# fernandezdaniel/MOBOCMF

Measured on AMD Instinct MI355X. Metric: ELBO steps/sec (MFDGP d=8 M=512 N=8192 S=8), higher is better.
Workload: dtype f64

## Files before the change

### mobocmf_amd/csrc/gram.hip

```cpp
#include "common.h"

#define GT 128
#define GM 32


typedef double v2f64_t __attribute__((ext_vector_type(2)));

template <int KIND, int DB, int XD>
__global__ __launch_bounds__(GT) void gram_fwd_kernel(GramArgs g) {
    __shared__ __attribute__((aligned(16))) double stg[XD ? (GT / 64) * 64 * (XD + 2) : 1];
    __shared__ double zs[GM][DB];
    __shared__ double zfs[GM];
    __shared__ double il1[DB], il2[DB];
    const int d = g.d;
    const int tid = threadIdx.x;
    const int gm = g.gm;
    const int m0 = blockIdx.y * gm;
    const double* hyp = g.hyp;
    double a1, af = 0, nu = 0, a2 = 0, ilf = 0;
    if (KIND == 0) {
        a1 = hyp[0];
        if (tid < DB) il1[tid] = tid < d ? 1.0 / hyp[1 + tid] : 0.0;
    } else {
        a1 = hyp[0]; af = hyp[1]; nu = hyp[2]; a2 = hyp[3]; ilf = 1.0 / hyp[4];
        if (tid < DB) { il1[tid] = tid < d ? 1.0 / hyp[5 + tid] : 0.0; il2[tid] = tid < d ? 1.0 / hyp[5 + d + tid] : 0.0; }
    }
    for (int e = tid; e < gm * DB; e += GT) {
        int mm = e / DB, k = e % DB;
        int m = m0 + mm;
        zs[mm][k] = (m < g.M && k < d) ? g.Zx[(int64_t)(m / g.zdiv) * d + k] : 0.0;
    }
    if (KIND == 1 && tid < gm) zfs[tid] = (m0 + tid < g.M) ? g.zf[m0 + tid] : 0.0;
    __syncthreads();

    const int64_t n0 = (int64_t)blockIdx.x * GT + tid;
    const int xdiv = XD ? XD : g.xdiv;
    const int64_t c0 = n0 * xdiv;
    if (c0 >= g.Np) return;
    const bool real = n0 < g.nbase;
    double xr[DB];
#pragma unroll
    for (int k = 0; k < DB; ++k) xr[k] = (real && k < d) ? g.x[n0 * d + k] : 0.0;
    double fr[XD ? XD : 1];
    if (XD && KIND == 1) {
#pragma unroll
        for (int s = 0; s < XD; s += 2) {
            v2f64_t v = real ? *(const v2f64_t*)(g.f + c0 + s) : (v2f64_t){0.0, 0.0};
            fr[s] = v[0];
            fr[s + 1] = v[1];
        }
    }

    const bool full_wave = XD && __ballot(real) == ~0ull;
    (void)full_wave;
    if (g.knn && blockIdx.y == 0) {
        for (int s = 0; s < xdiv; ++s) {
            int64_t n = c0 + s;
            if (n >= g.Np) break;
            double v = 0.0;
            if (real) {
                if (KIND == 0) v = a1;
                else { double fn = g.f[n]; v = a1 * (nu * fn * fn + af) + a2; }
            }
            g.knn[n] = v;
        }
    }
    for (int mm = 0; mm < gm; ++mm) {
        const int m = m0 + mm;
        double* krow = g.K + (int64_t)m * g.ldk;
        if (!real || m >= g.M) {
            for (int s = 0; s < xdiv; ++s) {
                int64_t n = c0 + s;
                if (n >= g.Np) break;
                krow[n] = (g.is_kmm && n == m) ? 1.0 : 0.0;
            }
            continue;
        }
        double d1 = 0.0, d2 = 0.0;
#pragma unroll
        for (int k = 0; k < DB; ++k) {
            double df = xr[k] - zs[mm][k];
            double t1 = df * il1[k];
            d1 += t1 * t1;
            if (KIND == 1) { double t2 = df * il2[k]; d2 += t2 * t2; }
        }
        const double E1 = exp(-0.5 * d1);
        if (KIND == 0) {
            double v = a1 * E1;
            if (g.is_kmm && c0 == m) v += g.jitter;
            krow[c0] = v;
            for (int s = 1; s < xdiv; ++s) krow[c0 + s] = a1 * E1;
        } else if (XD) {
            const double E2 = exp(-0.5 * d2);
            const double zfm = zfs[mm];
            const double c1 = a1 * E1, c2 = a2 * E2;
            const double cp = c1 * nu * zfm, cq = c1 * af;
            const int lane = tid & 63;
            double* my = stg + (tid >> 6) * 64 * (XD + 2);
#pragma unroll
            for (int s = 0; s < XD; s += 2) {
                v2f64_t v;
#pragma unroll
                for (int e = 0; e < 2; ++e) {
                    const double fn = fr[s + e];
                    const double fd = (fn - zfm) * ilf;
                    v[e] = cq * exp(-0.5 * fd * fd) + (cp * fn + c2);
                }
                if (full_wave) *(v2f64_t*)(my + lane * (XD + 2) + s) = v;
                else *(v2f64_t*)(krow + c0 + s) = v;
            }
            if (full_wave) {
                double* wrow = krow + (c0 - (int64_t)lane * XD);
#pragma unroll
                for (int i = 0; i < XD / 2; ++i) {
                    const int e = (i * 64 + lane) * 2;
                    *(v2f64_t*)(wrow + e) = *(const v2f64_t*)(my + (e / XD) * (XD + 2) + e % XD);
                }
            }
        } else {
            const double E2 = exp(-0.5 * d2);
            const double zfm = zfs[mm];
            const double c1 = a1 * E1, c2 = a2 * E2;
            for (int s = 0; s < xdiv; ++s) {
                const int64_t n = c0 + s;
                const double fn = g.f[n];
                const double fd = (fn - zfm) * ilf;
                const double Ef = exp(-0.5 * fd * fd);
                double v = c1 * (nu * fn * zfm + af * Ef) + c2;
                if (g.is_kmm && n == m) v += g.jitter;
                krow[n] = v;
            }
        }
    }
}

__device__ __forceinline__ double wave_sum(double v) {
    v += __shfl_xor(v, 1);
    v += __shfl_xor(v, 2);
    v += __shfl_xor(v, 4);
    v += __shfl_xor(v, 8);
    v += __shfl_xor(v, 16);
    v += __shfl_xor(v, 32);
    return v;
}

template <int KIND, int DB, bool WANT_DX, int XD>
__global__ __launch_bounds__(GT) void gram_bwd_kernel(GramArgs g) {
    __shared__ double zs[GM][DB];
    __shared__ double zfs[GM];
    __shared__ double il1[DB], il2[DB];
    __shared__ double dzf_s[GM];
    __shared__ double red[2][8 + 2 * DB];
    extern __shared__ double dfs[];
    const int d = g.d;
    const int tid = threadIdx.x, lane = tid & 63, wave = tid >> 6;
    const int gm = g.gm;
    const int m0 = blockIdx.y * gm;
    const double* hyp = g.hyp;
    double a1, af = 0, nu = 0, a2 = 0, ilf = 0;
    if (KIND == 0) {
        a1 = hyp[0];
        if (tid < DB) il1[tid] = tid < d ? 1.0 / hyp[1 + tid] : 0.0;
    } else {
        a1 = hyp[0]; af = hyp[1]; nu = hyp[2]; a2 = hyp[3]; ilf = 1.0 / hyp[4];
        if (tid < DB) { il1[tid] = tid < d ? 1.0 / hyp[5 + tid] : 0.0; il2[tid] = tid < d ? 1.0 / hyp[5 + d + tid] : 0.0; }
    }
    for (int e = tid; e < gm * DB; e += GT) {
        int mm = e / DB, k = e % DB;
        int m = m0 + mm;
        zs[mm][k] = (m < g.M && k < d) ? g.Zx[(int64_t)(m / g.zdiv) * d + k] : 0.0;
    }
    if (tid < gm) {
        dzf_s[tid] = 0.0;
        if (KIND == 1) zfs[tid] = (m0 + tid < g.M) ? g.zf[m0 + tid] : 0.0;
    }
    __syncthreads();

    const int64_t n0 = (int64_t)blockIdx.x * GT + tid;
    const int xdiv = XD ? XD : g.xdiv;
    const int64_t c0 = n0 * xdiv;
    const bool real = n0 < g.nbase;
    static_assert(XD == 0 || 128 % XD == 0, "replica runs must not straddle a column block");
    unsigned long long amask = ~0ull;
    if (g.colact && real) {
        if (XD) amask = g.colact[c0 >> 7] != 0 ? ~0ull : 0ull;
        else {
            amask = 0ull;
            for (int s = 0; s < xdiv; ++s) amask |= (unsigned long long)(g.colact[(c0 + s) >> 7] != 0 ? 1 : 0) << s;
        }
    }
    const bool live = real && amask != 0ull;
    double fr[XD ? XD : 1], dfa[XD ? XD : 1];
    if (XD) {
#pragma unroll
        for (int s = 0; s < XD; s += 2) {
            v2f64_t v = real ? *(const v2f64_t*)(g.f + c0 + s) : (v2f64_t){0.0, 0.0};
            fr[s] = v[0];
            fr[s + 1] = v[1];
            dfa[s] = dfa[s + 1] = 0.0;
        }
    }
    double xr[DB], aL1[DB], aL2[KIND == 1 ? DB : 1], aX[WANT_DX ? DB : 1];
#pragma unroll
    for (int k = 0; k < DB; ++k) {
        xr[k] = (real && k < d) ? g.x[n0 * d + k] : 0.0;
        aL1[k] = 0.0;
        if (KIND == 1) aL2[k] = 0.0;
        if (WANT_DX) aX[k] = 0.0;
    }
    double s_a1 = 0, s_af = 0, s_nu = 0, s_a2 = 0, s_lsf = 0;
    if (KIND == 1 && !XD)
        for (int s = 0; s < xdiv; ++s) dfs[s * GT + tid] = 0.0;

    if (g.gknn && blockIdx.y == 0 && real) {
        for (int s = 0; s < xdiv; ++s) {
            const int64_t n = c0 + s;
            const double gk = g.gknn[n];
            if (KIND == 0) s_a1 += gk;
            else {
                const double fn = g.f[n];
                s_a1 += gk * (nu * fn * fn + af);
                s_nu += gk * a1 * fn * fn;
                s_af += gk * a1;
                s_a2 += gk;
            }
        }
    }

    for (int mm = 0; mm < gm; ++mm) {
        const int m = m0 + mm;
        if (m >= g.M) break;
        double dzf_loc = 0.0;
        if (live) {
            const double* grow = g.G + (int64_t)m * g.ldk;
            double d1 = 0.0, d2 = 0.0;
#pragma unroll
            for (int k = 0; k < DB; ++k) {
                double df = xr[k] - zs[mm][k];
                double t1 = df * il1[k];
                d1 += t1 * t1;
                if (KIND == 1) { double t2 = df * il2[k]; d2 += t2 * t2; }
            }
            const double E1 = exp(-0.5 * d1);
            double W1 = 0.0, W2 = 0.0;
            if (KIND == 0) {
                double Gsum = 0.0;
                for (int s = 0; s < xdiv; ++s) Gsum += ((amask >> s) & 1ull) ? grow[c0 + s] : 0.0;
                s_a1 += Gsum * E1;
                W1 = Gsum * a1 * E1;
            } else {
                const double E2 = exp(-0.5 * d2);
                const double zfm = zfs[mm];
                const double aE1 = a1 * E1;
                const double c_a = aE1 * nu * zfm, c_b = aE1 * af * ilf;
                double G2s = 0.0, S1 = 0.0, S2 = 0.0, S3 = 0.0, S4 = 0.0;
                auto body = [&](double Gv, double fn, double& dfacc) {
                    const double fd = (fn - zfm) * ilf;
                    const double GEf = Gv * exp(-0.5 * fd * fd);
                    const double T = GEf * fd;
                    G2s += Gv;
                    S1 += Gv * fn;
                    S2 += GEf;
                    S3 += T;
                    S4 += T * fd;
                    dfacc += Gv * c_a - T * c_b;
                };
                if (XD) {
#pragma unroll
                    for (int s = 0; s < XD; s += 2) {
                        const v2f64_t Gp = *(const v2f64_t*)(grow + c0 + s);
                        body(Gp[0], fr[s], dfa[s]);
                        body(Gp[1], fr[s + 1], dfa[s + 1]);
                    }
                } else {
                    for (int s = 0; s < xdiv; ++s) {
                        double acc = 0.0;
                        body(((amask >> s) & 1ull) ? grow[c0 + s] : 0.0, g.f[c0 + s], acc);
                        dfs[s * GT + tid] += acc;
                    }
                }
                const double inner = nu * zfm * S1 + af * S2;
                s_a1 += E1 * inner;
                s_nu += aE1 * zfm * S1;
                s_af += aE1 * S2;
                s_lsf += c_b * S4;
                W1 = aE1 * inner;
                dzf_loc = aE1 * nu * S1 + c_b * S3;
                s_a2 += G2s * E2;
                W2 = G2s * a2 * E2;
            }
#pragma unroll
            for (int k = 0; k < DB; ++k) {
                double df = xr[k] - zs[mm][k];
                double t1 = df * il1[k];
                aL1[k] += W1 * t1 * t1;
                double gx = W1 * t1 * il1[k];
                if (KIND == 1) {
                    double t2 = df * il2[k];
                    aL2[k] += W2 * t2 * t2;
                    gx += W2 * t2 * il2[k];
                }
                if (WANT_DX) aX[k] -= gx;
            }
        }
        if (KIND == 1) {
            double tot = wave_sum(dzf_loc);
            if (lane == 0) atomicAdd(&dzf_s[mm], tot);
        }
    }
    if (KIND == 1) {
        for (int s = 0; s < xdiv; ++s) {
            const int64_t n = c0 + s;
            if (n >= g.Np) break;
            double v = real ? (XD ? dfa[XD ? s : 0] : dfs[s * GT + tid]) : 0.0;
            if (real && g.gknn && blockIdx.y == 0) v += g.gknn[n] * a1 * 2.0 * nu * g.f[n];
            g.df_part[(int64_t)blockIdx.y * g.Np + n] = v;
        }
    }
    if (WANT_DX && real) {
        double* dxp = g.dx_part + ((int64_t)blockIdx.y * g.nbase + n0) * d;
#pragma unroll
        for (int k = 0; k < DB; ++k)
            if (k < d) dxp[k] = aX[k];
    }
    const int H = (KIND == 0) ? 1 + d : 5 + 2 * d;
    {
        double v;
        v = wave_sum(s_a1); if (lane == 0) red[wave][0] = v;
        if (KIND == 1) {
            v = wave_sum(s_af); if (lane == 0) red[wave][1] = v;
            v = wave_sum(s_nu); if (lane == 0) red[wave][2] = v;
            v = wave_sum(s_a2); if (lane == 0) red[wave][3] = v;
            v = wave_sum(s_lsf); if (lane == 0) red[wave][4] = v;
        }
#pragma unroll
        for (int k = 0; k < DB; ++k) {
            if (k < d) {
                v = wave_sum(aL1[k]);
                if (lane == 0) red[wave][(KIND == 0 ? 1 : 5) + k] = v * il1[k];
                if (KIND == 1) {
                    v = wave_sum(aL2[k]);
                    if (lane == 0) red[wave][5 + d + k] = v * il2[k];
                }
            }
        }
    }
    __syncthreads();
    double* hp = g.hyp_part + ((int64_t)blockIdx.y * gridDim.x + blockIdx.x) * H;
    if (tid < H) hp[tid] = red[0][tid] + red[1][tid];
    if (KIND == 1 && tid < gm) g.dzf_part[(int64_t)blockIdx.x * g.Mp + m0 + tid] = dzf_s[tid];
}

__global__ void sum_partials_kernel(const double* part, int64_t P, int64_t stride, double* out, int64_t len,
                                    double scale, int accumulate) {
    int64_t j = (int64_t)blockIdx.x * blockDim.x + threadIdx.x;
    if (j >= len) return;
    double v = 0.0;
    for (int64_t p = 0; p < P; ++p) v += part[p * stride + j];
    v *= scale;
    out[j] = accumulate ? out[j] + v : v;
}

__global__ void sum_partials_wide_kernel(const double* part, int64_t P, int64_t stride, double* out, int64_t len,
                                         double scale, int accumulate) {
    __shared__ double sh[4];
    const int64_t j = blockIdx.x;
    double v = 0.0;
    for (int64_t p = threadIdx.x; p < P; p += 256) v += part[p * stride + j];
    v += __shfl_xor(v, 1); v += __shfl_xor(v, 2); v += __shfl_xor(v, 4);
    v += __shfl_xor(v, 8); v += __shfl_xor(v, 16); v += __shfl_xor(v, 32);
    if ((threadIdx.x & 63) == 0) sh[threadIdx.x >> 6] = v;
    __syncthreads();
    if (threadIdx.x == 0) {
        v = (sh[0] + sh[1] + sh[2] + sh[3]) * scale;
        out[j] = accumulate ? out[j] + v : v;
    }
}

__global__ void group_sum_kernel(const double* in, double* out, int64_t nout, int div, int accumulate) {
    int64_t j = (int64_t)blockIdx.x * blockDim.x + threadIdx.x;
    if (j >= nout) return;
    double v = 0.0;
    for (int s = 0; s < div; ++s) v += in[j * div + s];
    out[j] = accumulate ? out[j] + v : v;
}

#define SUM_MULTI_MAX 8
struct SumTasksArg { SumTask t[SUM_MULTI_MAX]; int blk0[SUM_MULTI_MAX + 1]; int wide[SUM_MULTI_MAX]; int n; };
__global__ void sum_partials_multi_kernel(SumTasksArg T) {
    __shared__ double sh[4];
    int k = 0;
    while (k + 1 < T.n && (int)blockIdx.x >= T.blk0[k + 1]) ++k;
    const SumTask& t = T.t[k];
    if (T.wide[k] == 1) {
        const int64_t j = (int64_t)(blockIdx.x - T.blk0[k]);
        double v = 0.0;
        for (int64_t p = threadIdx.x; p < t.P; p += 256) v += t.part[p * t.stride + j];
        if (t.part2)
            for (int64_t p = threadIdx.x; p < t.P2; p += 256) v += t.part2[p * t.stride2 + j];
        v += __shfl_xor(v, 1); v += __shfl_xor(v, 2); v += __shfl_xor(v, 4);
        v += __shfl_xor(v, 8); v += __shfl_xor(v, 16); v += __shfl_xor(v, 32);
        if ((threadIdx.x & 63) == 0) sh[threadIdx.x >> 6] = v;
        __syncthreads();
        if (threadIdx.x == 0) {
            v = sh[0] + sh[1] + sh[2] + sh[3];
            if (t.extra) v += t.extra[j];
            t.out[j] = t.accumulate ? t.out[j] + v : v;
        }
        return;
    }
    if (T.wide[k] == 2) {
        __shared__ double sq[4][64];
        const int jj = threadIdx.x & 63, q = threadIdx.x >> 6;
        const int64_t j = (int64_t)(blockIdx.x - T.blk0[k]) * 64 + jj;
        double v = 0.0;
        if (j < t.len) {
            for (int64_t p = q; p < t.P; p += 4) v += t.part[p * t.stride + j];
            if (t.part2)
                for (int64_t p = q; p < t.P2; p += 4) v += t.part2[p * t.stride2 + j];
        }
        sq[q][jj] = v;
        __syncthreads();
        if (q == 0 && j < t.len) {
            v = (sq[0][jj] + sq[1][jj]) + (sq[2][jj] + sq[3][jj]);
            if (t.extra) v += t.extra[j];
            t.out[j] = t.accumulate ? t.out[j] + v : v;
        }
        return;
    }
    const int64_t j = (int64_t)(blockIdx.x - T.blk0[k]) * blockDim.x + threadIdx.x;
    if (j >= t.len) return;
    double v = 0.0;
    for (int64_t p = 0; p < t.P; ++p) v += t.part[p * t.stride + j];
    if (t.part2)
        for (int64_t p = 0; p < t.P2; ++p) v += t.part2[p * t.stride2 + j];
    if (t.extra) v += t.extra[j];
    t.out[j] = t.accumulate ? t.out[j] + v : v;
}

int launch_sum_partials(const double* part, int64_t P, int64_t stride, double* out, int64_t len, double scale,
                        int accumulate, hipStream_t s);

int launch_sum_partials_multi(const SumTask* tasks, int n, hipStream_t s) {
    if (n > SUM_MULTI_MAX) {
        for (int i = 0; i < n; i += SUM_MULTI_MAX) {
            int rc = launch_sum_partials_multi(tasks + i, n - i < SUM_MULTI_MAX ? n - i : SUM_MULTI_MAX, s);
            if (rc) return rc;
        }
        return MOBOCMF_OK;
    }
    SumTasksArg T = {};
    int64_t nb = 0;
    int m = 0;
    for (int i = 0; i < n; ++i) {
        if (tasks[i].len <= 0) continue;
        T.t[m] = tasks[i];
        T.blk0[m] = (int)nb;
        const int64_t pmax = tasks[i].P > (tasks[i].part2 ? tasks[i].P2 : 0) ? tasks[i].P : tasks[i].P2;
        T.wide[m] = (pmax >= 64 && tasks[i].len <= 4096) ? 1 : (pmax >= 16 ? 2 : 0);
        nb += T.wide[m] == 1 ? tasks[i].len : T.wide[m] == 2 ? (tasks[i].len + 63) / 64 : (tasks[i].len + 255) / 256;
        ++m;
    }
    T.blk0[m] = (int)nb;
    T.n = m;
    if (m == 0) return MOBOCMF_OK;
    if (nb > 0x7fffffff) return MOBOCMF_BAD_ARG;
    hipLaunchKernelGGL(sum_partials_multi_kernel, dim3((unsigned)nb), dim3(256), 0, s, T);
    return hipGetLastError() == hipSuccess ? MOBOCMF_OK : MOBOCMF_HIP_ERROR;
}

int launch_sum_partials(const double* part, int64_t P, int64_t stride, double* out, int64_t len, double scale,
                        int accumulate, hipStream_t s) {
    if (len <= 0) return MOBOCMF_OK;
    if (P >= 64 && len <= 4096) {
        hipLaunchKernelGGL(sum_partials_wide_kernel, dim3((unsigned)len), dim3(256), 0, s, part, P, stride, out, len,
                           scale, accumulate);
        return hipGetLastError() == hipSuccess ? MOBOCMF_OK : MOBOCMF_HIP_ERROR;
    }
    hipLaunchKernelGGL(sum_partials_kernel, dim3((unsigned)((len + 255) / 256)), dim3(256), 0, s, part, P, stride, out,
                       len, scale, accumulate);
    return hipGetLastError() == hipSuccess ? MOBOCMF_OK : MOBOCMF_HIP_ERROR;
}

static inline int d_bucket(int d) { return d <= 2 ? 2 : (d <= 8 ? 8 : 32); }

static int gram_rows_per_block(const GramArgs& g, bool fwd = false) {
    int64_t nb_cols = (g.Np + g.xdiv - 1) / g.xdiv;
    int64_t gx = (nb_cols + GT - 1) / GT;
    int gm = GM;
    while (gm > GM / 4 && gx * (g.Mp / gm) < 1024) gm /= 2;
    if (fwd && g.is_kmm)
        while (gm > 2 && gx * (g.Mp / gm) < 4096) gm /= 2;
    return gm;
}
void gram_grid(const GramArgs& g, dim3* grid) {
    int64_t nb_cols = (g.Np + g.xdiv - 1) / g.xdiv;
    *grid = dim3((unsigned)((nb_cols + GT - 1) / GT), (unsigned)(g.Mp / gram_rows_per_block(g)), 1);
}

int launch_gram_fwd(const GramArgs& g0, hipStream_t s) {
    GramArgs g = g0;
    g.gm = gram_rows_per_block(g0, true);
    if (g.d < 1 || g.d > 32) return MOBOCMF_BAD_ARG;
    dim3 grid;
    gram_grid(g, &grid);
    grid.y = (unsigned)(g.Mp / g.gm);
    const int db = d_bucket(g.d);
#define GF(K, D, X) hipLaunchKernelGGL((gram_fwd_kernel<K, D, X>), grid, dim3(GT), 0, s, g)
    const bool vec_ok = g.kind == 1 && !g.is_kmm && ((uintptr_t)g.f % 16 == 0) && ((uintptr_t)g.K % 16 == 0) && (g.ldk % 2 == 0);
    if (g.kind == 0) { if (db == 2) GF(0, 2, 0); else if (db == 8) GF(0, 8, 0); else GF(0, 32, 0); }
    else if (vec_ok && g.xdiv == 8) { if (db == 2) GF(1, 2, 8); else if (db == 8) GF(1, 8, 8); else GF(1, 32, 8); }
    else if (vec_ok && g.xdiv == 16) { if (db == 2) GF(1, 2, 16); else if (db == 8) GF(1, 8, 16); else GF(1, 32, 16); }
    else { if (db == 2) GF(1, 2, 0); else if (db == 8) GF(1, 8, 0); else GF(1, 32, 0); }
#undef GF
    return hipGetLastError() == hipSuccess ? MOBOCMF_OK : MOBOCMF_HIP_ERROR;
}

int launch_gram_bwd(const GramArgs& g0, bool want_dx, hipStream_t s) {
    GramArgs g = g0;
    g.gm = gram_rows_per_block(g0);
    if (g.d < 1 || g.d > 32) return MOBOCMF_BAD_ARG;
    dim3 grid;
    gram_grid(g, &grid);
    const int db = d_bucket(g.d);
    if (g.xdiv > 48) return MOBOCMF_BAD_ARG;
    const size_t shm = g.kind == 1 ? (size_t)g.xdiv * GT * sizeof(double) : 0;
#define GB(K, D, X)                                                                                    \
    do {                                                                                               \
        if (want_dx) hipLaunchKernelGGL((gram_bwd_kernel<K, D, true, X>), grid, dim3(GT), (X) ? 0 : shm, s, g);   \
        else hipLaunchKernelGGL((gram_bwd_kernel<K, D, false, X>), grid, dim3(GT), (X) ? 0 : shm, s, g);          \
    } while (0)
    const bool vec_ok = g.kind == 1 && ((uintptr_t)g.f % 16 == 0) && ((uintptr_t)g.G % 16 == 0) && (g.ldk % 2 == 0);
    if (g.kind == 0) { if (db == 2) GB(0, 2, 0); else if (db == 8) GB(0, 8, 0); else GB(0, 32, 0); }
    else if (vec_ok && g.xdiv == 8) { if (db == 2) GB(1, 2, 8); else if (db == 8) GB(1, 8, 8); else GB(1, 32, 8); }
    else if (vec_ok && g.xdiv == 16) { if (db == 2) GB(1, 2, 16); else if (db == 8) GB(1, 8, 16); else GB(1, 32, 16); }
    else { if (db == 2) GB(1, 2, 0); else if (db == 8) GB(1, 8, 0); else GB(1, 32, 0); }
#undef GB
    return hipGetLastError() == hipSuccess ? MOBOCMF_OK : MOBOCMF_HIP_ERROR;
}
```

Baseline: 1065.

## Register-block gram kernels over inducing rows, prefetch G, and replace dzf atomics

```diff
diff --git a/mobocmf_amd/csrc/gram.hip b/mobocmf_amd/csrc/gram.hip
--- a/mobocmf_amd/csrc/gram.hip
+++ b/mobocmf_amd/csrc/gram.hip
@@ -1,7 +1,20 @@
-#include "common.h"
+#include <type_traits>
+
+#include "small_step_common.h"
 
 #define GT 128
 #define GM 32
+#define GMIN 4
+
+template <int KIND, int DB, int XD, bool WANT_DX = false>
+struct GramRowBlock {
+    static constexpr int fwd = KIND == 0 ? (DB == 32 ? 2 : 4) : ((DB == 32 || XD) ? 1 : 4);
+    static constexpr int bwd = KIND == 0 ? (DB == 32 ? 1 : 4)
+                               : XD ? 1
+                                    : (DB == 32 ? 1 : (DB == 8 ? (WANT_DX ? 1 : 2) : 4));
+    static constexpr bool bwd_prefetch = KIND == 0 ? DB < 32
+                                                   : (XD == 8 && DB <= 8 && !(WANT_DX && DB == 8)) || (XD == 16 && DB == 2);
+};
 
 
 typedef double v2f64_t __attribute__((ext_vector_type(2)));
@@ -65,83 +78,107 @@
             g.knn[n] = v;
         }
     }
-    for (int mm = 0; mm < gm; ++mm) {
-        const int m = m0 + mm;
-        double* krow = g.K + (int64_t)m * g.ldk;
-        if (!real || m >= g.M) {
+    if (!real) {
+        for (int mm = 0; mm < gm; ++mm) {
+            const int m = m0 + mm;
             for (int s = 0; s < xdiv; ++s) {
                 int64_t n = c0 + s;
                 if (n >= g.Np) break;
-                krow[n] = (g.is_kmm && n == m) ? 1.0 : 0.0;
-            }
-            continue;
-        }
-        double d1 = 0.0, d2 = 0.0;
-#pragma unroll
-        for (int k = 0; k < DB; ++k) {
-            double df = xr[k] - zs[mm][k];
-            double t1 = df * il1[k];
-            d1 += t1 * t1;
-            if (KIND == 1) { double t2 = df * il2[k]; d2 += t2 * t2; }
-        }
-        const double E1 = exp(-0.5 * d1);
+                g.K[(int64_t)m * g.ldk + n] = (g.is_kmm && n == m) ? 1.0 : 0.0;
+            }
+        }
+        return;
+    }
+    constexpr int RB = GramRowBlock<KIND, DB, XD>::fwd;
+    const int mv = g.M - m0 < gm ? (g.M - m0 > 0 ? g.M - m0 : 0) : gm;
+    auto rows = [&](auto RC, const int mm0) {
+        constexpr int R = decltype(RC)::value;
+        double E1[R], E2[R];
+#pragma unroll
+        for (int r = 0; r < R; ++r) {
+            double d1 = 0.0, d2 = 0.0;
+#pragma unroll
+            for (int k = 0; k < DB; ++k) {
+                double df = xr[k] - zs[mm0 + r][k];
+                double t1 = df * il1[k];
+                d1 += t1 * t1;
+                if (KIND == 1) { double t2 = df * il2[k]; d2 += t2 * t2; }
+            }
+            E1[r] = exp(-0.5 * d1);
+            E2[r] = KIND == 1 ? exp(-0.5 * d2) : 0.0;
+        }
         if (KIND == 0) {
-            double v = a1 * E1;
-            if (g.is_kmm && c0 == m) v += g.jitter;
-            krow[c0] = v;
-            for (int s = 1; s < xdiv; ++s) krow[c0 + s] = a1 * E1;
+#pragma unroll
+            for (int r = 0; r < R; ++r) {
+                const int m = m0 + mm0 + r;
+                double* krow = g.K + (int64_t)m * g.ldk;
+                double v = a1 * E1[r];
+                if (g.is_kmm && c0 == m) v += g.jitter;
+                krow[c0] = v;
+                for (int s = 1; s < xdiv; ++s) krow[c0 + s] = a1 * E1[r];
+            }
         } else if (XD) {
-            const double E2 = exp(-0.5 * d2);
-            const double zfm = zfs[mm];
-            const double c1 = a1 * E1, c2 = a2 * E2;
-            const double cp = c1 * nu * zfm, cq = c1 * af;
             const int lane = tid & 63;
             double* my = stg + (tid >> 6) * 64 * (XD + 2);
 #pragma unroll
-            for (int s = 0; s < XD; s += 2) {
-                v2f64_t v;
-#pragma unroll
-                for (int e = 0; e < 2; ++e) {
-                    const double fn = fr[s + e];
-                    const double fd = (fn - zfm) * ilf;
-                    v[e] = cq * exp(-0.5 * fd * fd) + (cp * fn + c2);
+            for (int r = 0; r < R; ++r) {
+                double* krow = g.K + (int64_t)(m0 + mm0 + r) * g.ldk;
+                const double zfm = zfs[mm0 + r];
+                const double c1 = a1 * E1[r], c2 = a2 * E2[r];
+                const double cp = c1 * nu * zfm, cq = c1 * af;
+#pragma unroll
+                for (int s = 0; s < XD; s += 2) {
+                    v2f64_t v;
+#pragma unroll
+                    for (int e = 0; e < 2; ++e) {
+                        const double fn = fr[s + e];
+                        const double fd = (fn - zfm) * ilf;
+                        v[e] = cq * exp(-0.5 * fd * fd) + (cp * fn + c2);
+                    }
+                    if (full_wave) *(v2f64_t*)(my + lane * (XD + 2) + s) = v;
+                    else *(v2f64_t*)(krow + c0 + s) = v;
                 }
-                if (full_wave) *(v2f64_t*)(my + lane * (XD + 2) + s) = v;
-                else *(v2f64_t*)(krow + c0 + s) = v;
-            }
-            if (full_wave) {
-                double* wrow = krow + (c0 - (int64_t)lane * XD);
-#pragma unroll
-                for (int i = 0; i < XD / 2; ++i) {
-                    const int e = (i * 64 + lane) * 2;
-                    *(v2f64_t*)(wrow + e) = *(const v2f64_t*)(my + (e / XD) * (XD + 2) + e % XD);
+                if (full_wave) {
+                    double* wrow = krow + (c0 - (int64_t)lane * XD);
+#pragma unroll
+                    for (int i = 0; i < XD / 2; ++i) {
+                        const int e = (i * 64 + lane) * 2;
+                        *(v2f64_t*)(wrow + e) = *(const v2f64_t*)(my + (e / XD) * (XD + 2) + e % XD);
+                    }
                 }
             }
         } else {
-            const double E2 = exp(-0.5 * d2);
-            const double zfm = zfs[mm];
-            const double c1 = a1 * E1, c2 = a2 * E2;
             for (int s = 0; s < xdiv; ++s) {
                 const int64_t n = c0 + s;
                 const double fn = g.f[n];
-                const double fd = (fn - zfm) * ilf;
-                const double Ef = exp(-0.5 * fd * fd);
-                double v = c1 * (nu * fn * zfm + af * Ef) + c2;
-                if (g.is_kmm && n == m) v += g.jitter;
-                krow[n] = v;
-            }
-        }
-    }
-}
-
-__device__ __forceinline__ double wave_sum(double v) {
-    v += __shfl_xor(v, 1);
-    v += __shfl_xor(v, 2);
-    v += __shfl_xor(v, 4);
-    v += __shfl_xor(v, 8);
-    v += __shfl_xor(v, 16);
-    v += __shfl_xor(v, 32);
-    return v;
+#pragma unroll
+                for (int r = 0; r < R; ++r) {
+                    const int m = m0 + mm0 + r;
+                    const double zfm = zfs[mm0 + r];
+                    const double c1 = a1 * E1[r], c2 = a2 * E2[r];
+                    const double fd = (fn - zfm) * ilf;
+                    const double Ef = exp(-0.5 * fd * fd);
+                    double v = c1 * (nu * fn * zfm + af * Ef) + c2;
+                    if (g.is_kmm && n == m) v += g.jitter;
+                    g.K[(int64_t)m * g.ldk + n] = v;
+                }
+            }
+        }
+    };
+    int mm = 0;
+#pragma nounroll
+    for (; mm + RB <= mv; mm += RB) rows(std::integral_constant<int, RB>{}, mm);
+    if (RB > 1)
+#pragma nounroll
+        for (; mm < mv; ++mm) rows(std::integral_constant<int, 1>{}, mm);
+    for (; mm < gm; ++mm) {
+        const int m = m0 + mm;
+        for (int s = 0; s < xdiv; ++s) {
+            int64_t n = c0 + s;
+            if (n >= g.Np) break;
+            g.K[(int64_t)m * g.ldk + n] = (g.is_kmm && n == m) ? 1.0 : 0.0;
+        }
+    }
 }
 
 template <int KIND, int DB, bool WANT_DX, int XD>
@@ -149,7 +186,7 @@
     __shared__ double zs[GM][DB];
     __shared__ double zfs[GM];
     __shared__ double il1[DB], il2[DB];
-    __shared__ double dzf_s[GM];
+    __shared__ double dzl[KIND == 1 ? GM : 1][KIND == 1 ? GT + 4 : 1];
     __shared__ double red[2][8 + 2 * DB];
     extern __shared__ double dfs[];
     const int d = g.d;
@@ -170,10 +207,7 @@
         int m = m0 + mm;
         zs[mm][k] = (m < g.M && k < d) ? g.Zx[(int64_t)(m / g.zdiv) * d + k] : 0.0;
     }
-    if (tid < gm) {
-        dzf_s[tid] = 0.0;
-        if (KIND == 1) zfs[tid] = (m0 + tid < g.M) ? g.zf[m0 + tid] : 0.0;
-    }
+    if (KIND == 1 && tid < gm) zfs[tid] = (m0 + tid < g.M) ? g.zf[m0 + tid] : 0.0;
     __syncthreads();
 
     const int64_t n0 = (int64_t)blockIdx.x * GT + tid;
@@ -227,86 +261,151 @@
         }
     }
 
-    for (int mm = 0; mm < gm; ++mm) {
-        const int m = m0 + mm;
-        if (m >= g.M) break;
-        double dzf_loc = 0.0;
-        if (live) {
-            const double* grow = g.G + (int64_t)m * g.ldk;
+    constexpr int RB = GramRowBlock<KIND, DB, XD, WANT_DX>::bwd;
+    constexpr int PF = KIND == 0 ? 1 : (XD ? XD : 1);
+    constexpr bool HOLDS_G = KIND == 0 || XD > 0;
+    constexpr bool PREFETCH = GramRowBlock<KIND, DB, XD, WANT_DX>::bwd_prefetch;
+    const int mv = g.M - m0 < gm ? (g.M - m0 > 0 ? g.M - m0 : 0) : gm;
+    auto loadG = [&](auto RC, const int mm0, double (*Gb)[PF]) {
+        constexpr int R = decltype(RC)::value;
+#pragma unroll
+        for (int r = 0; r < R; ++r) {
+            const double* grow = g.G + (int64_t)(m0 + mm0 + r) * g.ldk;
+            if (KIND == 0) {
+                double Gsum = 0.0;
+                for (int s = 0; s < xdiv; ++s) Gsum += ((amask >> s) & 1ull) ? grow[c0 + s] : 0.0;
+                Gb[r][0] = Gsum;
+            } else if (XD) {
+#pragma unroll
+                for (int s = 0; s < XD; s += 2) {
+                    const v2f64_t Gp = *(const v2f64_t*)(grow + c0 + s);
+                    Gb[r][XD ? s : 0] = Gp[0];
+                    Gb[r][XD ? s + 1 : 0] = Gp[1];
+                }
+            }
+        }
+    };
+    auto rows = [&](auto RC, const int mm0, const double (*Gb)[PF]) {
+        constexpr int R = decltype(RC)::value;
+        double E1[R], E2[R], W1[R], W2[R];
+#pragma unroll
+        for (int r = 0; r < R; ++r) {
             double d1 = 0.0, d2 = 0.0;
 #pragma unroll
             for (int k = 0; k < DB; ++k) {
-                double df = xr[k] - zs[mm][k];
+                double df = xr[k] - zs[mm0 + r][k];
                 double t1 = df * il1[k];
                 d1 += t1 * t1;
                 if (KIND == 1) { double t2 = df * il2[k]; d2 += t2 * t2; }
             }
-            const double E1 = exp(-0.5 * d1);
-            double W1 = 0.0, W2 = 0.0;
-            if (KIND == 0) {
-                double Gsum = 0.0;
-                for (int s = 0; s < xdiv; ++s) Gsum += ((amask >> s) & 1ull) ? grow[c0 + s] : 0.0;
-                s_a1 += Gsum * E1;
-                W1 = Gsum * a1 * E1;
+            E1[r] = exp(-0.5 * d1);
+            E2[r] = KIND == 1 ? exp(-0.5 * d2) : 0.0;
+            W2[r] = 0.0;
+        }
+        if (KIND == 0) {
+#pragma unroll
+            for (int r = 0; r < R; ++r) {
+                const double Gsum = Gb[r][0];
+                s_a1 += Gsum * E1[r];
+                W1[r] = Gsum * a1 * E1[r];
+            }
+        } else {
+            double zfm[R], aE1[R], c_a[R], c_b[R], G2s[R], S1[R], S2[R], S3[R], S4[R];
+#pragma unroll
+            for (int r = 0; r < R; ++r) {
+                zfm[r] = zfs[mm0 + r];
+                aE1[r] = a1 * E1[r];
+                c_a[r] = aE1[r] * nu * zfm[r];
+                c_b[r] = aE1[r] * af * ilf;
+                G2s[r] = S1[r] = S2[r] = S3[r] = S4[r] = 0.0;
+            }
+            auto body = [&](const int r, double Gv, double fn, double& dfacc) {
+                const double fd = (fn - zfm[r]) * ilf;
+                const double GEf = Gv * exp(-0.5 * fd * fd);
+                const double T = GEf * fd;
+                G2s[r] += Gv;
+                S1[r] += Gv * fn;
+                S2[r] += GEf;
+                S3[r] += T;
+                S4[r] += T * fd;
+                dfacc += Gv * c_a[r] - T * c_b[r];
+            };
+            if (XD) {
+#pragma unroll
+                for (int r = 0; r < R; ++r)
+#pragma unroll
+                    for (int s = 0; s < XD; ++s) body(r, Gb[r][XD ? s : 0], fr[XD ? s : 0], dfa[XD ? s : 0]);
             } else {
-                const double E2 = exp(-0.5 * d2);
-                const double zfm = zfs[mm];
-                const double aE1 = a1 * E1;
-                const double c_a = aE1 * nu * zfm, c_b = aE1 * af * ilf;
-                double G2s = 0.0, S1 = 0.0, S2 = 0.0, S3 = 0.0, S4 = 0.0;
-                auto body = [&](double Gv, double fn, double& dfacc) {
-                    const double fd = (fn - zfm) * ilf;
-                    const double GEf = Gv * exp(-0.5 * fd * fd);
-                    const double T = GEf * fd;
-                    G2s += Gv;
-                    S1 += Gv * fn;
-                    S2 += GEf;
-                    S3 += T;
-                    S4 += T * fd;
-                    dfacc += Gv * c_a - T * c_b;
-                };
-                if (XD) {
-#pragma unroll
-                    for (int s = 0; s < XD; s += 2) {
-                        const v2f64_t Gp = *(const v2f64_t*)(grow + c0 + s);
-                        body(Gp[0], fr[s], dfa[s]);
-                        body(Gp[1], fr[s + 1], dfa[s + 1]);
+                for (int s = 0; s < xdiv; ++s) {
+                    const bool on = (amask >> s) & 1ull;
+                    const double fn = g.f[c0 + s];
+                    double dsum = dfs[s * GT + tid];
+#pragma unroll
+                    for (int r = 0; r < R; ++r) {
+                        double acc = 0.0;
+                        body(r, on ? g.G[(int64_t)(m0 + mm0 + r) * g.ldk + c0 + s] : 0.0, fn, acc);
+                        dsum += acc;
                     }
-                } else {
-                    for (int s = 0; s < xdiv; ++s) {
-                        double acc = 0.0;
-                        body(((amask >> s) & 1ull) ? grow[c0 + s] : 0.0, g.f[c0 + s], acc);
-                        dfs[s * GT + tid] += acc;
-                    }
+                    dfs[s * GT + tid] = dsum;
                 }
-                const double inner = nu * zfm * S1 + af * S2;
-                s_a1 += E1 * inner;
-                s_nu += aE1 * zfm * S1;
-                s_af += aE1 * S2;
-                s_lsf += c_b * S4;
-                W1 = aE1 * inner;
-                dzf_loc = aE1 * nu * S1 + c_b * S3;
-                s_a2 += G2s * E2;
-                W2 = G2s * a2 * E2;
-            }
+            }
+#pragma unroll
+            for (int r = 0; r < R; ++r) {
+                const double inner = nu * zfm[r] * S1[r] + af * S2[r];
+                s_a1 += E1[r] * inner;
+                s_nu += aE1[r] * zfm[r] * S1[r];
+                s_af += aE1[r] * S2[r];
+                s_lsf += c_b[r] * S4[r];
+                W1[r] = aE1[r] * inner;
+                dzl[KIND == 1 ? mm0 + r : 0][KIND == 1 ? tid : 0] = aE1[r] * nu * S1[r] + c_b[r] * S3[r];
+                s_a2 += G2s[r] * E2[r];
+                W2[r] = G2s[r] * a2 * E2[r];
+            }
+        }
+#pragma unroll
+        for (int r = 0; r < R; ++r) {
 #pragma unroll
             for (int k = 0; k < DB; ++k) {
-                double df = xr[k] - zs[mm][k];
+                double df = xr[k] - zs[mm0 + r][k];
                 double t1 = df * il1[k];
-                aL1[k] += W1 * t1 * t1;
-                double gx = W1 * t1 * il1[k];
+                aL1[k] += W1[r] * t1 * t1;
+                double gx = W1[r] * t1 * il1[k];
                 if (KIND == 1) {
                     double t2 = df * il2[k];
-                    aL2[k] += W2 * t2 * t2;
-                    gx += W2 * t2 * il2[k];
+                    aL2[k] += W2[r] * t2 * t2;
+                    gx += W2[r] * t2 * il2[k];
                 }
                 if (WANT_DX) aX[k] -= gx;
             }
         }
-        if (KIND == 1) {
-            double tot = wave_sum(dzf_loc);
-            if (lane == 0) atomicAdd(&dzf_s[mm], tot);
-        }
+    };
+    if (live) {
+        using RBc = std::integral_constant<int, RB>;
+        using R1c = std::integral_constant<int, 1>;
+        const int nfull = mv / RB * RB;
+        double Gc[RB][PF], Gn[RB][PF];
+        if (PREFETCH && nfull > 0) loadG(RBc{}, 0, Gc);
+#pragma nounroll
+        for (int mm = 0; mm < nfull; mm += RB) {
+            if (PREFETCH) {
+                if (mm + RB < nfull) loadG(RBc{}, mm + RB, Gn);
+            } else if (HOLDS_G) loadG(RBc{}, mm, Gc);
+            rows(RBc{}, mm, Gc);
+            if (PREFETCH) {
+#pragma unroll
+                for (int r = 0; r < RB; ++r)
+#pragma unroll
+                    for (int s = 0; s < PF; ++s) Gc[r][s] = Gn[r][s];
+            }
+        }
+#pragma nounroll
+        for (int mm = nfull; RB > 1 && mm < mv; ++mm) {
+            double G1[1][PF];
+            if (HOLDS_G) loadG(R1c{}, mm, G1);
+            rows(R1c{}, mm, G1);
+        }
+    } else if (KIND == 1) {
+        for (int mm = 0; mm < mv; ++mm) dzl[KIND == 1 ? mm : 0][KIND == 1 ? tid : 0] = 0.0;
     }
     if (KIND == 1) {
         for (int s = 0; s < xdiv; ++s) {
@@ -326,21 +425,21 @@
     const int H = (KIND == 0) ? 1 + d : 5 + 2 * d;
     {
         double v;
-        v = wave_sum(s_a1); if (lane == 0) red[wave][0] = v;
+        v = wsum63(s_a1); if (lane == 63) red[wave][0] = v;
         if (KIND == 1) {
-            v = wave_sum(s_af); if (lane == 0) red[wave][1] = v;
-            v = wave_sum(s_nu); if (lane == 0) red[wave][2] = v;
-            v = wave_sum(s_a2); if (lane == 0) red[wave][3] = v;
-            v = wave_sum(s_lsf); if (lane == 0) red[wave][4] = v;
+            v = wsum63(s_af); if (lane == 63) red[wave][1] = v;
+            v = wsum63(s_nu); if (lane == 63) red[wave][2] = v;
+            v = wsum63(s_a2); if (lane == 63) red[wave][3] = v;
+            v = wsum63(s_lsf); if (lane == 63) red[wave][4] = v;
         }
 #pragma unroll
         for (int k = 0; k < DB; ++k) {
             if (k < d) {
-                v = wave_sum(aL1[k]);
-                if (lane == 0) red[wave][(KIND == 0 ? 1 : 5) + k] = v * il1[k];
+                v = wsum63(aL1[k]);
+                if (lane == 63) red[wave][(KIND == 0 ? 1 : 5) + k] = v * il1[k];
                 if (KIND == 1) {
-                    v = wave_sum(aL2[k]);
-                    if (lane == 0) red[wave][5 + d + k] = v * il2[k];
+                    v = wsum63(aL2[k]);
+                    if (lane == 63) red[wave][5 + d + k] = v * il2[k];
                 }
             }
         }
@@ -348,7 +447,15 @@
     __syncthreads();
     double* hp = g.hyp_part + ((int64_t)blockIdx.y * gridDim.x + blockIdx.x) * H;
     if (tid < H) hp[tid] = red[0][tid] + red[1][tid];
-    if (KIND == 1 && tid < gm) g.dzf_part[(int64_t)blockIdx.x * g.Mp + m0 + tid] = dzf_s[tid];
+    if (KIND == 1) {
+        const int r = tid >> 2, q = tid & 3;
+        double v = 0.0;
+        if (r < mv)
+            for (int i = 0; i < GT / 4; ++i) v += dzl[KIND == 1 ? r : 0][KIND == 1 ? i * 4 + q : 0];
+        v += __shfl_xor(v, 1);
+        v += __shfl_xor(v, 2);
+        if (q == 0 && r < gm) g.dzf_part[(int64_t)blockIdx.x * g.Mp + m0 + r] = v;
+    }
 }
 
 __global__ void sum_partials_kernel(const double* part, int64_t P, int64_t stride, double* out, int64_t len,
@@ -488,9 +595,9 @@
     int64_t nb_cols = (g.Np + g.xdiv - 1) / g.xdiv;
     int64_t gx = (nb_cols + GT - 1) / GT;
     int gm = GM;
-    while (gm > GM / 4 && gx * (g.Mp / gm) < 1024) gm /= 2;
+    while (gm > GMIN && gx * (g.Mp / gm) < 1024) gm /= 2;
     if (fwd && g.is_kmm)
-        while (gm > 2 && gx * (g.Mp / gm) < 4096) gm /= 2;
+        while (gm > GMIN && gx * (g.Mp / gm) < 4096) gm /= 2;
     return gm;
 }
 void gram_grid(const GramArgs& g, dim3* grid) {
```

Result: no change. 1072, median of 6 (+0.7%).
